# mschoenb97/po2_quantization

Measured on AMD Instinct MI355X. Metric: quantized-conv fwd images/sec, ResNet56 224×224 bs=256; 1/2/4/8 MI355X, higher is better.
Workload: dtype fp32(bf16x3); 1 GPU; resnet56 quantized-conv chain: 56 fused po2-4bit quantize+conv fwd + head (stage-1 and stage-2 conv1->conv2 pairs as one launch each) (stride-2 conv1 + 1x1 shortcut of stages 2-3 as one launch each) (weight packs of the single-conv layers batched: one launch per 36); conv_pairs=True, conv_pairs_stage2=True, s2ds=True, pack_batch=True, autotune=True, image=224, batch_per_gpu=256, global_batch=256, quantizer=po2, bits=4, precision=bf16x3, parallelism=dp1, world_size=1, hip_graph=False

## Files before the change

### po2_quantization_amd/csrc/po2q_conv_rowsk.hip

```cpp
#include <hip/hip_runtime.h>

#include <algorithm>
#include <climits>
#include <cstdlib>
#include <type_traits>
#include <vector>

#include "po2q_epi.h"
#include "po2q_internal.h"
#include "po2q_quant_dev.h"
#include "po2q_rows_dev.h"
#include "po2q_x3_dev.h"

namespace po2q {

namespace {

constexpr int kKSW = 32;
constexpr int kKWC = kKSW + 2;
template <int C> constexpr int kKPlane = kKWC * C * 2;
template <int C> constexpr int kKRawInt = C * kKSW * 4;
template <int C> constexpr int kKRawSlot = kKRawInt<C> + 4 * 256;
template <int C> constexpr int kKTile = C * kKSW * 4;
template <int C, int PD, bool TT>
constexpr int kKLds = 2 * 3 * kKPlane<C> + PD * kKRawSlot<C> + (TT ? 2 * kKTile<C> : 0);

template <int C>
__device__ __forceinline__ int k_addr(int hc, int oct) {
    if constexpr (C == 64)
        return hc * 128 + ((oct ^ (hc & 7)) << 4);
    else
        return x_addr<32>(hc, oct);
}

}

struct RowsKArgs {
    int N, H, W, P, Q;
    int RB, nseg, nstrip, items;
    int remap;
    const float* ps;
    const float* pb;
    int act;
    const float* res;
    WQuant q;
};

template <int C, int PD, bool TT, bool RES, bool NTL>
__device__ __forceinline__ void loader_wave(const float* __restrict__ x, const RowsKArgs& a, unsigned char* raw,
                                            unsigned char* resb, int n, int q0, int p0, int nrows, int rbe) {
    constexpr int NI = C / 8 + 1;
    static_assert(2 * C <= 64, "one halo instruction per row");
    const int lane = threadIdx.x & 63;
    const int HW = a.H * a.W;
    const uint32_t cstride = (uint32_t)HW * 4u;
    const __amdgpu_buffer_rsrc_t rs = rows_rsrc(x + (int64_t)n * C * HW, C * HW * 4);
    const int gq4 = q0 + 4 * (lane & 7);
    const bool qi_ok = gq4 < a.W;
    const uint32_t vi0 = (uint32_t)(lane >> 3) * cstride + (uint32_t)gq4 * 4u;
    const int hside = lane / C, hch = lane % C;
    const int gqh = hside ? q0 + kKSW : q0 - 1;
    const bool qh_ok = gqh >= 0 && gqh < a.W;
    const uint32_t vh0 = (uint32_t)hch * cstride + (uint32_t)gqh * 4u;
    const uint32_t raw_lds = (uint32_t)(uintptr_t)raw;
    const int PQ = a.P * a.Q;
    const __amdgpu_buffer_rsrc_t rr = rows_rsrc(RES ? a.res + (int64_t)n * C * PQ : x, RES ? C * PQ * 4 : 4);
    const uint32_t vr0 = (uint32_t)(lane >> 3) * (uint32_t)PQ * 4u + (uint32_t)gq4 * 4u;
    auto lres = [&](int js) __attribute__((always_inline)) {
        const int orow = js - 3;
        const bool ok = orow >= 0 && orow < rbe && gq4 < a.Q;
        const uint32_t vo = ok ? vr0 + (uint32_t)(p0 + orow) * (uint32_t)a.Q * 4u : 0x7fffffffu;
        const uint32_t base = (uint32_t)(uintptr_t)resb + (uint32_t)((js & 1) * kKTile<C>);
#pragma unroll
        for (int i = 0; i < C / 8; ++i) rows_dma16(rr, vo, i * 8u * (uint32_t)PQ * 4u, base + (uint32_t)i * 1024u);
    };
    auto lrow = [&](int sl, int j) __attribute__((always_inline)) {
        const int h = p0 - 1 + j;
        const bool hok = j < nrows && h >= 0 && h < a.H;
        const uint32_t roff = (uint32_t)(hok ? h : 0) * (uint32_t)a.W * 4u;
        const uint32_t vo = (hok && qi_ok) ? vi0 + roff : 0x7fffffffu;
        const uint32_t base = raw_lds + (uint32_t)(sl * kKRawSlot<C>);
#pragma unroll
        for (int i = 0; i < C / 8; ++i) rows_dma16<NTL>(rs, vo, i * 8u * cstride, base + (uint32_t)i * 1024u);
        rows_dma4<NTL>(rs, (hok && qh_ok) ? vh0 + roff : 0x7fffffffu, base + (uint32_t)kKRawInt<C>);
    };
#pragma unroll
    for (int r = 0; r < PD; ++r) lrow(r, r);
    rows_wait<(PD - 1) * NI>();
    __builtin_amdgcn_s_barrier();
    const int steps = (nrows + 2) / 3 * 3;
    int sl = 0;
    for (int j = 0; j < steps; ++j) {
        rows_wait<(PD - 2) * NI>();
        __builtin_amdgcn_s_barrier();
        if constexpr (RES) lres(j + 1);
        lrow(sl, j + PD);
        sl = sl + 1 == PD ? 0 : sl + 1;
    }
    if (TT && nrows % 3 == 0) {
        if constexpr (RES) rows_wait<0>();
        __builtin_amdgcn_s_barrier();
    }
    asm volatile("s_waitcnt vmcnt(0)" ::: "memory");
}

template <int C, int PD, bool TT, bool LW, bool EPI = false, int DBG = 0, int NTS = 0, bool RES = false,
          bool FP = false, bool PIPE = false>
__global__ __launch_bounds__(LW ? kThreads + 64 : kThreads, C == 64 ? (TT ? 2 : 3) : 4) void conv_rowsk(const float* __restrict__ x, const uint4* __restrict__ wpk,
                                                          const float* __restrict__ scale_p,
                                                          const float* __restrict__ bias, float* __restrict__ y,
                                                          RowsKArgs a) {
    static_assert(!PIPE || (!LW && !RES && !FP && DBG == 0), "pipelined split: plain MFMA-wave plans");
#ifndef PO2Q_ROWSK_FPF
#define PO2Q_ROWSK_FPF 0
#endif
    constexpr bool FPF = PO2Q_ROWSK_FPF != 0 && TT;
    constexpr int K = C;
    constexpr int NCH = C / 32;
    constexpr int KSC = 3 * NCH;
    constexpr int WN = K / 16;
    constexpr int NGW = 2 * WN / 4;
    constexpr int DPW = C / 32;
    constexpr int HPW = C / 2;
    constexpr int PL = kKPlane<C>;
    constexpr int RAWI = kKRawInt<C>;
    constexpr int RAWS = kKRawSlot<C>;
    extern __shared__ __attribute__((aligned(16))) unsigned char lds[];
    const int tid = threadIdx.x, lane = tid & 63;
    const int wave = __builtin_amdgcn_readfirstlane(tid >> 6);
    const int wn = wave % WN;
    const int g0 = (wave / WN) * NGW;
    unsigned char* planes = lds;
    unsigned char* raw = lds + 2 * 3 * PL;
    unsigned char* tile = raw + PD * kKRawSlot<C>;
    unsigned char* resb = tile + 2 * kKTile<C>;

    int blk = blockIdx.x;
    if (a.remap) blk = (blk & 7) * (int)(gridDim.x >> 3) + (blk >> 3);
    const int item = blk;
    if (item >= a.items) return;
    const int strip = item % a.nstrip;
    const int t0 = item / a.nstrip;
    const int seg = t0 % a.nseg;
    const int n = t0 / a.nseg;
    const int q0 = strip * kKSW;
    const int p0 = seg * a.RB;
    const int rbe = min(a.RB, a.P - p0);
    const int nrows = rbe + 2;

    if constexpr (LW) {
        if (wave == 4) {
            loader_wave<C, PD, TT, RES, (NTS & 2) != 0>(x, a, raw, resb, n, q0, p0, nrows, rbe);
            return;
        }
    }

    static_assert(!(FP && LW), "the loader wave keeps its own barrier count");
    bf16x8 bw[3][KSC];
    float scale;
    if constexpr (FP) {
        unsigned* red = reinterpret_cast<unsigned*>(raw);
        unsigned* thr = red + 16;
        bool fin;
        scale = wq_prologue(a.q, thr, red, 4, fin);
        uint4* fr = reinterpret_cast<uint4*>(planes);
        static_assert(KSC * WN * 64 * 16 <= 2 * 3 * PL, "fragment scratch in the planes");
#pragma unroll
        for (int r = 0; r < 3; ++r) {
            wq_pack_tap_row_lds<C>(a.q, C, 32, WN, KSC, r, scale, fin, thr, fr);
#pragma unroll
            for (int ks = 0; ks < KSC; ++ks) bw[r][ks] = __builtin_bit_cast(bf16x8, fr[(ks * WN + wn) * 64 + lane]);
            __syncthreads();
        }
    } else {
#pragma unroll
        for (int r = 0; r < 3; ++r)
#pragma unroll
            for (int ks = 0; ks < KSC; ++ks)
                bw[r][ks] = __builtin_bit_cast(bf16x8, wpk[((r * KSC + ks) * WN + wn) * 64 + lane]);
        scale = *scale_p;
    }
    const int kout = 16 * wn + (lane & 15);
    float bk = bias ? bias[kout] : 0.0f;
    float eps_ = (EPI && a.ps) ? a.ps[kout] : 1.0f;
    float epb_ = (EPI && a.pb) ? a.pb[kout] : 0.0f;
#pragma unroll
    for (int r = 0; r < 3; ++r)
#pragma unroll
        for (int ks = 0; ks < KSC; ++ks) asm volatile("s_waitcnt vmcnt(0)" : "+v"(bw[r][ks]));
    asm volatile("s_waitcnt vmcnt(0)" : "+v"(bk), "+v"(eps_), "+v"(epb_));
    auto outv = [&](float accv) __attribute__((always_inline)) {
        const float v = accv * scale + bk;
        if constexpr (EPI && RES)
            return v * eps_ + epb_;
        else if constexpr (EPI)
            return epi_act(v * eps_ + epb_, a.act);
        else
            return v;
    };

    const int HW = a.H * a.W;
    const uint32_t cstride = (uint32_t)HW * 4u;
    const __amdgpu_buffer_rsrc_t rs = rows_rsrc(x + (int64_t)n * C * HW, C * HW * 4);
    const int cb = lane & 7;
    const int gq4 = q0 + 4 * cb;
    const bool qi_ok = gq4 < a.W;
    const uint32_t vi0 = (uint32_t)((C / 4) * wave + (lane >> 3)) * cstride + (uint32_t)gq4 * 4u;
    const uint32_t soff1 = 8u * cstride;
    const int hv = HPW * wave + lane;
    const int hside = hv / C, hch = hv % C;
    const int gqh = hside ? q0 + kKSW : q0 - 1;
    const bool qh_ok = lane < HPW && gqh >= 0 && gqh < a.W;
    const uint32_t vh0 = (uint32_t)hch * cstride + (uint32_t)gqh * 4u;
    const uint32_t raw_lds = (uint32_t)(uintptr_t)raw;

    const int sc = lane & 31, so = lane >> 5;
    const bool sl_ok = so < DPW;
    const int oct = DPW * wave + (sl_ok ? so : 0);
    const int rd0 = (8 * oct) * (kKSW * 4) + sc * 4;
    const int wa_i = k_addr<C>(sc + 1, oct);
    const int wa_h = k_addr<C>(hside ? kKWC - 1 : 0, hch >> 3) + (hch & 7) * 2;

    int aoff[NGW][KSC];
    {
        const int p = lane & 15, g = lane >> 4;
#pragma unroll
        for (int grp = 0; grp < NGW; ++grp)
#pragma unroll
            for (int ch = 0; ch < NCH; ++ch)
#pragma unroll
                for (int s = 0; s < 3; ++s)
                    aoff[grp][ch * 3 + s] = k_addr<C>(16 * (g0 + grp) + p + s, 4 * ch + g);
    }

    auto load_row = [&](auto SL_, int j) __attribute__((always_inline)) {
        constexpr int sl = decltype(SL_)::value;
        const int h = p0 - 1 + j;
        const bool hok = j < nrows && h >= 0 && h < a.H;
        const uint32_t roff = (uint32_t)(hok ? h : 0) * (uint32_t)a.W * 4u;
        const uint32_t vo = (hok && qi_ok && !(DBG & 8)) ? vi0 + roff : 0x7fffffffu;
        const uint32_t voh = (hok && qh_ok && !(DBG & 1)) ? vh0 + roff : 0x7fffffffu;
        const uint32_t base = raw_lds + (uint32_t)(sl * RAWS);
#pragma unroll
        for (int i = 0; i < DPW; ++i) rows_dma16<(NTS & 2) != 0>(rs, vo, i * soff1, base + (uint32_t)(DPW * wave + i) * 1024u);
        rows_dma4<(NTS & 2) != 0>(rs, voh, base + (uint32_t)RAWI + (uint32_t)wave * 256u);
    };
    constexpr int NR = (RES && !LW) ? NGW : 0;
    static_assert(!RES || TT, "the residual rides on the TT output tile");
    constexpr int VMW = (PD - 1) * (NR + DPW + 1 + NGW) + NGW;
    constexpr int RW = 2 * (DPW + 1) + NGW + NR;
    const int PQ = a.P * a.Q;
    const __amdgpu_buffer_rsrc_t rres = rows_rsrc(NR ? a.res + (int64_t)n * K * PQ : x, NR ? K * PQ * 4 : 4);
    const uint32_t vr0 = (uint32_t)((K / 4) * wave + (lane >> 3)) * (uint32_t)PQ * 4u + (uint32_t)gq4 * 4u;
    auto load_res = [&](int js) __attribute__((always_inline)) {
        if constexpr (NR != 0) {
            const int orow = js - 3;
            const bool ok = orow >= 0 && orow < rbe && gq4 < a.Q;
            const uint32_t vo = ok ? vr0 + (uint32_t)(p0 + orow) * (uint32_t)a.Q * 4u : 0x7fffffffu;
            const uint32_t base = (uint32_t)(uintptr_t)resb + (uint32_t)((js & 1) * kKTile<C>) +
                                  (uint32_t)((K / 4) * wave) * (kKSW * 4u);
#pragma unroll
            for (int i = 0; i < NR; ++i) rows_dma16(rres, vo, i * 8u * (uint32_t)PQ * 4u, base + (uint32_t)i * 1024u);
        }
    };
    const __amdgpu_buffer_rsrc_t ry = rows_rsrc(y + (int64_t)n * K * PQ, K * PQ * 4);

    auto store_tile = [&](const unsigned char* tr, int o, bool orow, int rslot) __attribute__((always_inline)) {
        const int sb = lane & 7;
        const int q = q0 + 4 * sb;
#pragma unroll
        for (int i = 0; i < NGW; ++i) {
            const int c = (K / 4) * wave + 8 * i + (lane >> 3);
            floatx4 v = floatx4{0.f, 0.f, 0.f, 0.f};
            if constexpr (!(DBG & 256)) v = *reinterpret_cast<const floatx4*>(tr + c * (kKSW * 4) + ((sb ^ (c & 7)) << 4));
            if constexpr (RES) {
                const floatx4 r = *reinterpret_cast<const floatx4*>(resb + rslot * kKTile<C> + c * (kKSW * 4) + 16 * sb);
#pragma unroll
                for (int e = 0; e < 4; ++e) v[e] = epi_act(v[e] + r[e], a.act);
            }
            const uint32_t vo = (uint32_t)c * (uint32_t)PQ + (uint32_t)(orow ? o : 0) * a.Q + (uint32_t)q;
            rows_store<(NTS & 1) != 0 || (DBG & 32) != 0>(ry, (orow && q < a.Q && !(DBG & 16)) ? vo * 4u : 0x7fffffffu, v);
        }
    };

    auto split_row = [&](const unsigned char* rw, unsigned char* pb) __attribute__((always_inline)) {
        uint32_t b8[8];
#pragma unroll
        for (int e = 0; e < 8; ++e) b8[e] = *reinterpret_cast<const uint32_t*>(rw + rd0 + e * (kKSW * 4));
        uint4 hi, mid, lo;
        split3(b8, hi, mid, lo);
        if (sl_ok) {
            *reinterpret_cast<uint4*>(pb + wa_i) = hi;
            *reinterpret_cast<uint4*>(pb + PL + wa_i) = mid;
            *reinterpret_cast<uint4*>(pb + 2 * PL + wa_i) = lo;
        }
        if (lane < HPW) {
            uint16_t h16, m16, l16;
            const int hoff = LW ? 4 * (HPW * wave + lane) : wave * 256 + 4 * lane;
            split1(*reinterpret_cast<const uint32_t*>(rw + RAWI + hoff), h16, m16, l16);
            *reinterpret_cast<uint16_t*>(pb + wa_h) = h16;
            *reinterpret_cast<uint16_t*>(pb + PL + wa_h) = m16;
            *reinterpret_cast<uint16_t*>(pb + 2 * PL + wa_h) = l16;
        }
    };

    floatx4 acc[3][NGW];
#pragma unroll
    for (int sl = 0; sl < 3; ++sl)
#pragma unroll
        for (int grp = 0; grp < NGW; ++grp) acc[sl][grp] = floatx4{0.f, 0.f, 0.f, 0.f};

    auto step = [&](auto S_, int j) __attribute__((always_inline)) {
        constexpr int S6 = decltype(S_)::value;
        constexpr int S = S6 % 3;
        constexpr int B2 = S6 % 2;
        constexpr int RS = S6 % PD;
        unsigned char* pb = planes + B2 * 3 * PL;
        [[maybe_unused]] const unsigned char* rw = raw + RS * RAWS;
        if constexpr (LW || PIPE) {
        } else if constexpr (DBG & 64) {
            rows_wait<31>();
        } else {
            rows_wait<VMW>();
        }
        if constexpr (!PIPE) {
            if constexpr (!(DBG & 4)) split_row(rw, pb);
            asm volatile("s_waitcnt lgkmcnt(0)" ::: "memory");
            __builtin_amdgcn_s_barrier();
            if constexpr (!(DBG & 128) && !LW) {
                load_res(j + 1);
                load_row(std::integral_constant<int, RS>{}, j + PD);
            }
        }
        auto fin = [&]() __attribute__((always_inline)) {
            if constexpr (PIPE) {
                asm volatile("s_waitcnt lgkmcnt(0)" ::: "memory");
                __builtin_amdgcn_s_barrier();
                load_row(std::integral_constant<int, (S6 + 1) % PD>{}, j + 1 + PD);
            }
        };
        constexpr int SL[3] = {(S + 1) % 3, S, (S + 2) % 3};
        auto mma = [&](auto G_, auto&& after0) __attribute__((always_inline)) {
            constexpr bool G = decltype(G_)::value;
            bf16x8 af[2][3][NGW];
            auto ldf = [&](bf16x8 (&f)[3][NGW], int ks) __attribute__((always_inline)) {
#pragma unroll
                for (int pl = 0; pl < 3; ++pl)
#pragma unroll
                    for (int grp = 0; grp < NGW; ++grp)
                        f[pl][grp] = __builtin_bit_cast(bf16x8, *reinterpret_cast<const uint4*>(pb + pl * PL + aoff[grp][ks]));
            };
            if constexpr (FPF && !(DBG & 2)) ldf(af[0], 0);
#pragma unroll
            for (int ks = 0; ks < KSC && !(DBG & 2); ++ks) {
                bf16x8 (&cf)[3][NGW] = af[FPF ? (ks & 1) : 0];
                if constexpr (FPF) {
                    if (ks + 1 < KSC) ldf(af[(ks + 1) & 1], ks + 1);
                } else {
                    ldf(cf, ks);
                }
#pragma unroll
                for (int rr = 0; rr < 3; ++rr) {
                    if (G && (j - rr < 0 || j - rr >= rbe)) continue;
#pragma unroll
                    for (int pl = 0; pl < 3; ++pl)
#pragma unroll
                        for (int grp = 0; grp < NGW; ++grp)
                            acc[SL[rr]][grp] = __builtin_amdgcn_mfma_f32_16x16x32_bf16(cf[pl][grp], bw[rr][ks],
                                                                                      acc[SL[rr]][grp], 0, 0, 0);
                }
                if (ks == 0) after0();
            }
        };
        if constexpr (PIPE) {
            auto nxt = [&]() __attribute__((always_inline)) {
                rows_wait<(PD - 1) * (DPW + 1 + NGW)>();
                split_row(raw + ((S6 + 1) % PD) * RAWS, planes + (1 - B2) * 3 * PL);
            };
            if (j >= 2 && j < rbe)
                mma(std::false_type{}, nxt);
            else
                mma(std::true_type{}, nxt);
        } else {
            auto none = []() __attribute__((always_inline)) {};
            if (j >= 2 && j < rbe)
                mma(std::false_type{}, none);
            else
                mma(std::true_type{}, none);
        }
        constexpr int D = (S + 2) % 3;
        if constexpr (TT) {
            if constexpr (NR != 0) rows_wait<RW>();
            store_tile(tile + (1 - B2) * kKTile<C>, p0 + j - 3, j >= 3 && j - 3 < rbe, B2);
            unsigned char* tw = tile + B2 * kKTile<C>;
#pragma unroll
            for (int grp = 0; grp < NGW; ++grp) {
                floatx4 v;
                v[0] = outv(acc[D][grp][0]);
                v[1] = outv(acc[D][grp][1]);
                v[2] = outv(acc[D][grp][2]);
                v[3] = outv(acc[D][grp][3]);
                const int bi = 4 * (g0 + grp) + (lane >> 4);
                if constexpr (!(DBG & 256))
                    *reinterpret_cast<floatx4*>(tw + kout * (kKSW * 4) + ((bi ^ (kout & 7)) << 4)) = v;
                acc[D][grp] = floatx4{0.f, 0.f, 0.f, 0.f};
            }
            fin();
            return;
        }
        const int o = p0 + j - 2;
        const bool orow = j >= 2 && o < p0 + rbe;
        const uint32_t yk = (uint32_t)kout * (uint32_t)PQ + (uint32_t)(orow ? o : 0) * a.Q;
#pragma unroll
        for (int grp = 0; grp < NGW; ++grp) {
            const int q = q0 + 16 * (g0 + grp) + 4 * (lane >> 4);
            floatx4 v;
            v[0] = outv(acc[D][grp][0]);
            v[1] = outv(acc[D][grp][1]);
            v[2] = outv(acc[D][grp][2]);
            v[3] = outv(acc[D][grp][3]);
            rows_store<(NTS & 1) != 0>(ry, (orow && q < a.Q && !(DBG & 16)) ? (yk + (uint32_t)q) * 4u : 0x7fffffffu, v);
            acc[D][grp] = floatx4{0.f, 0.f, 0.f, 0.f};
        }
        fin();
    };

    {
        const floatx4 z = floatx4{0.f, 0.f, 0.f, 0.f};
        auto pre = [&](auto R_) __attribute__((always_inline)) {
            load_res(decltype(R_)::value - PD + 1);
            load_row(R_, decltype(R_)::value);
#pragma unroll
            for (int i = 0; i < NGW; ++i) rows_store<(NTS & 1) != 0>(ry, 0x7fffffffu, z);
        };
        if constexpr (LW) {
            __builtin_amdgcn_s_barrier();
        } else {
            pre(std::integral_constant<int, 0>{});
            pre(std::integral_constant<int, 1>{});
            if constexpr (PD >= 3) pre(std::integral_constant<int, 2>{});
            if constexpr (PIPE) {
                rows_wait<VMW>();
                split_row(raw, planes);
                asm volatile("s_waitcnt lgkmcnt(0)" ::: "memory");
                __builtin_amdgcn_s_barrier();
                load_row(std::integral_constant<int, 0>{}, PD);
            }
        }
    }
    for (int j = 0; j < nrows; j += 6) {
        step(std::integral_constant<int, 0>{}, j);
        step(std::integral_constant<int, 1>{}, j + 1);
        step(std::integral_constant<int, 2>{}, j + 2);
        if (j + 3 >= nrows) break;
        step(std::integral_constant<int, 3>{}, j + 3);
        step(std::integral_constant<int, 4>{}, j + 4);
        step(std::integral_constant<int, 5>{}, j + 5);
    }
    if (TT && nrows % 3 == 0) {
        if constexpr (NR != 0) rows_wait<0>();
        asm volatile("s_waitcnt lgkmcnt(0)" ::: "memory");
        __builtin_amdgcn_s_barrier();
        store_tile(tile + ((nrows - 1) & 1) * kKTile<C>, p0 + rbe - 1, true, nrows & 1);
    }
    asm volatile("s_waitcnt vmcnt(0)" ::: "memory");
}

static int rowsk_lds(int C, int pd, bool tt) {
#define PO2Q_L(c, d) \
    if (C == c && pd == d) return tt ? kKLds<c, d, true> : kKLds<c, d, false>;
    PO2Q_L(64, 2) PO2Q_L(64, 3) PO2Q_L(32, 2) PO2Q_L(32, 3)
#undef PO2Q_L
    return 1 << 30;
}

void rowsk_candidates(const ConvPlan& b, int mode, int bits, int fsr, std::vector<PlanCand>& out) {
    if (mode == 0 || b.groups != 1) return;
    if (bits < 1 || bits > 16) return;
    const long lo = (long)fsr - (1L << (bits - 1)), hi = (long)fsr - 1;
    if (lo < -126 || hi > 127) return;
    if (b.R != 3 || b.S != 3 || b.sh != 1 || b.sw != 1 || b.ph != 1 || b.pw != 1 || b.dh != 1 || b.dw != 1) return;
    if (!((b.C == 64 && b.K == 64) || (b.C == 32 && b.K == 32)) || b.Q % 4 != 0) return;
    if ((int64_t)b.C * b.H * b.W * 4 >= (1LL << 31) || (int64_t)b.K * b.P * b.Q * 4 >= (1LL << 31)) return;
    ConvPlan p = b;
    p.kind = KIND_BF16X3_ROWS;
    p.vrx = 1;
    p.CC = 32;
    p.nchunks = b.C / 32;
    p.NT = b.K / 16;
    p.NJ = 2;
    p.TQ = kKSW;
    p.steps = 3 * p.nchunks;
    p.kblocks = 1;
    p.taps = 9;
    p.PS = 0; p.MI = 0; p.pd = 2;
    p.dma_d0 = p.dma_nck = p.dma_ni = p.dma_nw = p.dma_waves = p.dma_ov = 0;
    p.HH = 0; p.WW = p.WWp = kKWC;
    p.SB = 2 * b.C;
    p.plane = b.C == 64 ? kKPlane<64> : kKPlane<32>;
    p.packed_floats = (int64_t)3 * p.steps * p.NT * 64 * 4;
    p.tilesQ = (p.Q + kKSW - 1) / kKSW;
    const int vrxs[3] = {b.C == 64 ? 1 : 3, 2, b.C == 64 ? 0 : 1};
    for (int vrx : vrxs)
        for (int pd : {3, 2}) {
            if (vrx == 0 || (vrx == 3 && pd < 3)) continue;
            ConvPlan c = p;
            c.pd = pd;
            c.vrx = vrx;
            const bool tt = vrx >= 2;
            c.lds_bytes = rowsk_lds(b.C, pd, tt);
            const int per_cu = std::min(b.C == 64 ? (tt ? 2 : 3) : 4, (int)(163840 / c.lds_bytes));
            const int slots = 256 * per_cu;
            std::vector<std::pair<double, int>> rbs;
            for (int rb = 4; rb <= p.P; ++rb) {
                const int nseg = (p.P + rb - 1) / rb;
                if (rb != (p.P + nseg - 1) / nseg) continue;
                const int64_t items = (int64_t)p.N * nseg * p.tilesQ;
                if (items > INT_MAX / 2) continue;
                rbs.push_back({(double)((items + slots - 1) / slots) * (rb + 2), rb});
            }
            std::sort(rbs.begin(), rbs.end());
            for (int i = 0; i < (int)rbs.size() && i < 2; ++i) {
                ConvPlan d = c;
                d.TP = rbs[i].second;
                d.tilesP = (p.P + d.TP - 1) / d.TP;
                const int64_t items = (int64_t)p.N * d.tilesP * d.tilesQ;
                d.blocks = (items + 7) / 8 * 8;
                out.push_back({0.9 + 0.001 * i + (pd == 2 ? 0.01 : 0.0) + (vrx == vrxs[0] ? 0.0 : 0.02), d});
                if (b.C == 64 && vrx == 1) {
                    ConvPlan f = d;
                    f.fp = 1;
                    out.push_back({0.95 + 0.001 * i + (pd == 2 ? 0.01 : 0.0), f});
                }
                if ((b.C == 64 && vrx == 1) || (b.C == 32 && vrx == 3))
                    for (int nts : {1, 2, 3}) {
                        d.nts = nts;
                        out.push_back({0.905 + 0.001 * i + 0.0001 * nts + (pd == 2 ? 0.01 : 0.0), d});
                    }
            }
        }
}

hipError_t launch_conv_rowsk(const ConvPlan& p, const float* x, const uint16_t* packed, const float* scale,
                             const float* bias, float* y, hipStream_t s, const float* ps, const float* pb,
                             int act, bool epi, const WQuant& q) {
    RowsKArgs a;
    a.N = p.N; a.H = p.H; a.W = p.W; a.P = p.P; a.Q = p.Q;
    a.RB = p.TP; a.nseg = p.tilesP; a.nstrip = p.tilesQ;
    a.items = p.N * p.tilesP * p.tilesQ;
    a.remap = (p.blocks % 8 == 0) ? 1 : 0;
    a.ps = ps;
    a.pb = pb;
    a.act = act;
    a.res = nullptr;
    a.q = q;
    if (p.fp) {
        if (!q.w || p.vrx != 1 || p.C != 64 || p.nts) return hipErrorInvalidValue;
#define PO2Q_RKF(d, e)                                                                                     \
    if (p.pd == d && epi == e) {                                                                             \
        hipLaunchKernelGGL((conv_rowsk<64, d, false, false, e, 0, 0, false, true>), dim3((unsigned)p.blocks), \
                           dim3(kThreads), p.lds_bytes, s, x, reinterpret_cast<const uint4*>(packed), scale, bias, y, a); \
        return hipGetLastError();                                                                            \
    }
        PO2Q_RKF(3, false) PO2Q_RKF(2, false) PO2Q_RKF(3, true) PO2Q_RKF(2, true)
#undef PO2Q_RKF
        return hipErrorInvalidValue;
    }
#define PO2Q_RK1(c, d, e, v, tt, lw)                                                                      \
    if (p.C == c && p.pd == d && epi == e && p.vrx == v && !p.nts) {                                         \
        hipLaunchKernelGGL((conv_rowsk<c, d, tt, lw, e>), dim3((unsigned)p.blocks), dim3(kThreads + (lw ? 64 : 0)), \
                           p.lds_bytes, s, x, reinterpret_cast<const uint4*>(packed), scale, bias, y, a);     \
        return hipGetLastError();                                                                            \
    }
#define PO2Q_RKN1(c, d, e, v, tt, lw, nt)                                                                 \
    if (p.C == c && p.pd == d && epi == e && p.vrx == v && p.nts == nt) {                                    \
        hipLaunchKernelGGL((conv_rowsk<c, d, tt, lw, e, 0, nt>), dim3((unsigned)p.blocks),                  \
                           dim3(kThreads + (lw ? 64 : 0)), p.lds_bytes, s, x, reinterpret_cast<const uint4*>(packed), \
                           scale, bias, y, a);                                                               \
        return hipGetLastError();                                                                            \
    }
#define PO2Q_RKN(c, d, e, v, tt, lw) \
    PO2Q_RKN1(c, d, e, v, tt, lw, 1) PO2Q_RKN1(c, d, e, v, tt, lw, 2) PO2Q_RKN1(c, d, e, v, tt, lw, 3)
#define PO2Q_RK(c, d, e) PO2Q_RK1(c, d, e, 1, false, false) PO2Q_RK1(c, d, e, 2, true, false)
    const int pipe = [] {
        const char* e = getenv("PO2Q_ROWSK_PIPE");
        return e ? atoi(e) : -1;
    }();
#define PO2Q_RKP(d, e, v, tt)                                                                                \
    if ((pipe == 1 || (pipe < 0 && v == 1)) && p.C == 64 && p.pd == d && epi == e && p.vrx == v && !p.nts) { \
        hipLaunchKernelGGL((conv_rowsk<64, d, tt, false, e, 0, 0, false, false, true>), dim3((unsigned)p.blocks), \
                           dim3(kThreads), p.lds_bytes, s, x, reinterpret_cast<const uint4*>(packed), scale, bias, y, a); \
        return hipGetLastError();                                                                            \
    }
    PO2Q_RKP(2, false, 2, true) PO2Q_RKP(3, false, 2, true) PO2Q_RKP(2, true, 2, true) PO2Q_RKP(3, true, 2, true)
    PO2Q_RKP(2, false, 1, false) PO2Q_RKP(3, false, 1, false) PO2Q_RKP(2, true, 1, false) PO2Q_RKP(3, true, 1, false)
#undef PO2Q_RKP
#define PO2Q_RKPN1(d, e, nt)                                                                                 \
    if (pipe != 0 && p.C == 64 && p.pd == d && epi == e && p.vrx == 1 && p.nts == nt) {                      \
        hipLaunchKernelGGL((conv_rowsk<64, d, false, false, e, 0, nt, false, false, true>), dim3((unsigned)p.blocks), \
                           dim3(kThreads), p.lds_bytes, s, x, reinterpret_cast<const uint4*>(packed), scale, bias, y, a); \
        return hipGetLastError();                                                                            \
    }
#define PO2Q_RKPN(d, e) PO2Q_RKPN1(d, e, 1) PO2Q_RKPN1(d, e, 2) PO2Q_RKPN1(d, e, 3)
    PO2Q_RKPN(2, false) PO2Q_RKPN(3, false) PO2Q_RKPN(2, true) PO2Q_RKPN(3, true)
#undef PO2Q_RKPN
#undef PO2Q_RKPN1
#ifdef PO2Q_ROWS_DIAG
    if (const char* dv = getenv("PO2Q_ROWSK_DEBUG")) {
        const int dbg = atoi(dv);
#define PO2Q_RKD(c, d, tt, lw, v)                                                                          \
    if (dbg == v && p.C == c && p.pd == d && (p.vrx >= 2) == tt && (p.vrx == 3) == lw) {                   \
        hipLaunchKernelGGL((conv_rowsk<c, d, tt, lw, false, v>), dim3((unsigned)p.blocks), dim3(kThreads + (lw ? 64 : 0)), \
                           p.lds_bytes, s, x, reinterpret_cast<const uint4*>(packed), scale, bias, y, a);    \
        return hipGetLastError();                                                                           \
    }
#define PO2Q_RKDS(v) PO2Q_RKD(32, 3, true, false, v) PO2Q_RKD(32, 3, true, true, v)
        PO2Q_RKDS(6) PO2Q_RKDS(16) PO2Q_RKDS(2) PO2Q_RKDS(1) PO2Q_RKDS(7)
#undef PO2Q_RKDS
#define PO2Q_RKDS(v) PO2Q_RKD(64, 2, true, false, v)
        PO2Q_RKDS(2) PO2Q_RKDS(4) PO2Q_RKDS(6) PO2Q_RKDS(16) PO2Q_RKDS(64) PO2Q_RKDS(128) PO2Q_RKDS(256)
        PO2Q_RKDS(144) PO2Q_RKDS(400) PO2Q_RKDS(404) PO2Q_RKDS(148) PO2Q_RKDS(20) PO2Q_RKDS(132)
#undef PO2Q_RKDS
#undef PO2Q_RKD
    }
#endif
    PO2Q_RK(64, 3, false) PO2Q_RK(64, 2, false) PO2Q_RK(32, 3, false) PO2Q_RK(32, 2, false)
    PO2Q_RK(64, 3, true) PO2Q_RK(64, 2, true) PO2Q_RK(32, 3, true) PO2Q_RK(32, 2, true)
    PO2Q_RK1(32, 3, false, 3, true, true) PO2Q_RK1(32, 3, true, 3, true, true)
    PO2Q_RKN(64, 3, false, 1, false, false) PO2Q_RKN(64, 2, false, 1, false, false)
    PO2Q_RKN(64, 3, true, 1, false, false) PO2Q_RKN(64, 2, true, 1, false, false)
    PO2Q_RKN(32, 3, false, 3, true, true) PO2Q_RKN(32, 3, true, 3, true, true)

#undef PO2Q_RK
#undef PO2Q_RK1
#undef PO2Q_RKN
#undef PO2Q_RKN1
    return hipErrorInvalidValue;
}

static bool rowsk64_res_on() {
    static const bool on = [] {
        const char* e = getenv("PO2Q_ROWSK_RES");
        return !(e && e[0] == '0');
    }();
    return on;
}

bool rowsk_res_ok(const ConvPlan& p) {
    if (p.kind != KIND_BF16X3_ROWS) return false;
    if (p.C == 32 && p.K == 32) return p.vrx == 3 && p.pd == 3 && !p.fp;
    return p.C == 64 && p.K == 64 && (p.vrx == 1 || p.vrx == 2) && rowsk64_res_on();
}

hipError_t launch_conv_rowsk_res(const ConvPlan& p, const float* x, const uint16_t* packed, const float* scale,
                                 const float* bias, float* y, const float* ps, const float* pb, const float* res,
                                 int act, hipStream_t s, const WQuant& q) {
    if (!rowsk_res_ok(p) || !res) return hipErrorInvalidValue;
    RowsKArgs a;
    a.N = p.N; a.H = p.H; a.W = p.W; a.P = p.P; a.Q = p.Q;
    a.RB = p.TP; a.nseg = p.tilesP; a.nstrip = p.tilesQ;
    a.items = p.N * p.tilesP * p.tilesQ;
    a.remap = (p.blocks % 8 == 0) ? 1 : 0;
    a.ps = ps;
    a.pb = pb;
    a.act = act;
    a.res = res;
    a.q = q;
    if (p.C == 64) {
        constexpr size_t lds64 = kKLds<64, 2, true> + 2 * kKTile<64>;
        if (p.fp) {
            if (!q.w) return hipErrorInvalidValue;
            hipLaunchKernelGGL((conv_rowsk<64, 2, true, false, true, 0, 0, true, true>), dim3((unsigned)p.blocks),
                               dim3(kThreads), lds64, s, x, reinterpret_cast<const uint4*>(packed), scale, bias, y, a);
        } else {
            hipLaunchKernelGGL((conv_rowsk<64, 2, true, false, true, 0, 0, true>), dim3((unsigned)p.blocks),
                               dim3(kThreads), lds64, s, x, reinterpret_cast<const uint4*>(packed), scale, bias, y, a);
        }
        return hipGetLastError();
    }
    const size_t lds = p.lds_bytes + 2 * kKTile<32>;
#define PO2Q_RKR(nt)                                                                                         \
    if (p.nts == nt) {                                                                                       \
        hipLaunchKernelGGL((conv_rowsk<32, 3, true, true, true, 0, nt, true>), dim3((unsigned)p.blocks),      \
                           dim3(kThreads + 64), lds, s, x, reinterpret_cast<const uint4*>(packed), scale, bias, y, a); \
        return hipGetLastError();                                                                            \
    }
    PO2Q_RKR(1) PO2Q_RKR(2) PO2Q_RKR(3)
#undef PO2Q_RKR
    if (p.nts != 0) return hipErrorInvalidValue;
    hipLaunchKernelGGL((conv_rowsk<32, 3, true, true, true, 0, 0, true>), dim3((unsigned)p.blocks),
                       dim3(kThreads + 64), lds, s, x, reinterpret_cast<const uint4*>(packed), scale, bias, y, a);
    return hipGetLastError();
}

}
```

Before: 26250 images/s.

## Add 64-column strip variant of rows conv kernel for C=64 stage-3 layers

Adds an SW=64 template path where a single block covers the full output width (Q between 33 and 64) for C=64 convolutions. It drops the halo loads and uses a new raw-slot layout, bf16x3 split and zeroed plane borders. Matching autotune candidates get a favourable prior cost, and the residual launcher now computes its own strip count. The intent is to cut redundant halo traffic and the per-strip weight-load overhead, at the price of more LDS per block and lower occupancy.

```diff
diff --git a/po2_quantization_amd/csrc/po2q_conv_rowsk.hip b/po2_quantization_amd/csrc/po2q_conv_rowsk.hip
--- a/po2_quantization_amd/csrc/po2q_conv_rowsk.hip
+++ b/po2_quantization_amd/csrc/po2q_conv_rowsk.hip
@@ -24,6 +24,9 @@
 template <int C> constexpr int kKTile = C * kKSW * 4;
 template <int C, int PD, bool TT>
 constexpr int kKLds = 2 * 3 * kKPlane<C> + PD * kKRawSlot<C> + (TT ? 2 * kKTile<C> : 0);
+constexpr int kKRawWave64 = 16 * 64 * 4;
+constexpr int kKRawSlot64 = 4 * kKRawWave64;
+constexpr int rowsk_lds64(int Q, int pd) { return 2 * 3 * (Q + 2) * 128 + pd * kKRawSlot64; }
 
 template <int C>
 __device__ __forceinline__ int k_addr(int hc, int oct) {
@@ -37,6 +40,7 @@
 
 struct RowsKArgs {
     int N, H, W, P, Q;
+    int QR;
     int RB, nseg, nstrip, items;
     int remap;
     const float* ps;
@@ -105,12 +109,20 @@
 }
 
 template <int C, int PD, bool TT, bool LW, bool EPI = false, int DBG = 0, int NTS = 0, bool RES = false,
-          bool FP = false, bool PIPE = false>
-__global__ __launch_bounds__(LW ? kThreads + 64 : kThreads, C == 64 ? (TT ? 2 : 3) : 4) void conv_rowsk(const float* __restrict__ x, const uint4* __restrict__ wpk,
+          bool FP = false, bool PIPE = false, int SW = 32>
+__global__ __launch_bounds__(LW ? kThreads + 64 : kThreads, SW == 64 ? 2 : C == 64 ? (TT ? 2 : 3) : 4) void conv_rowsk(const float* __restrict__ x, const uint4* __restrict__ wpk,
                                                           const float* __restrict__ scale_p,
                                                           const float* __restrict__ bias, float* __restrict__ y,
                                                           RowsKArgs a) {
-    static_assert(!PIPE || (!LW && !RES && !FP && DBG == 0), "pipelined split: plain MFMA-wave plans");
+    constexpr bool W64 = SW == 64;
+    static_assert(SW == 32 || SW == 64, "strip width");
+    static_assert(!PIPE || (!LW && !RES && !FP && (DBG == 0 || W64)), "pipelined split: plain MFMA-wave plans");
+    static_assert(!W64 || (C == 64 && PIPE), "64-column strips: C = 64, pipelined split");
+    static_assert(!W64 || !TT, "64-column strips store directly");
+    static_assert(!W64 || !LW, "64-column strips: no loader wave");
+    static_assert(!W64 || !RES, "64-column strips: no residual ring");
+    static_assert(!W64 || !FP, "64-column strips: packed weights only");
+    static_assert(!W64 || (DBG & ~(2 | 8 | 16)) == 0, "64-column strips: DBG 2, 8, 16");
 #ifndef PO2Q_ROWSK_FPF
 #define PO2Q_ROWSK_FPF 0
 #endif
@@ -119,20 +131,22 @@
     constexpr int NCH = C / 32;
     constexpr int KSC = 3 * NCH;
     constexpr int WN = K / 16;
-    constexpr int NGW = 2 * WN / 4;
-    constexpr int DPW = C / 32;
+    constexpr int NGW = (SW / 16) * WN / 4;
+    constexpr int DPW = W64 ? 4 : C / 32;
+    constexpr int HD = W64 ? 0 : 1;
     constexpr int HPW = C / 2;
-    constexpr int PL = kKPlane<C>;
+    constexpr int PLC = kKPlane<C>;
+    const int PL = W64 ? (a.QR + 2) * 128 : PLC;
     constexpr int RAWI = kKRawInt<C>;
-    constexpr int RAWS = kKRawSlot<C>;
+    constexpr int RAWS = W64 ? kKRawSlot64 : kKRawSlot<C>;
     extern __shared__ __attribute__((aligned(16))) unsigned char lds[];
     const int tid = threadIdx.x, lane = tid & 63;
     const int wave = __builtin_amdgcn_readfirstlane(tid >> 6);
     const int wn = wave % WN;
-    const int g0 = (wave / WN) * NGW;
+    const int g0 = W64 ? 0 : (wave / WN) * NGW;
     unsigned char* planes = lds;
     unsigned char* raw = lds + 2 * 3 * PL;
-    unsigned char* tile = raw + PD * kKRawSlot<C>;
+    unsigned char* tile = raw + PD * RAWS;
     unsigned char* resb = tile + 2 * kKTile<C>;
 
     int blk = blockIdx.x;
@@ -143,7 +157,7 @@
     const int t0 = item / a.nstrip;
     const int seg = t0 % a.nseg;
     const int n = t0 / a.nseg;
-    const int q0 = strip * kKSW;
+    const int q0 = strip * SW;
     const int p0 = seg * a.RB;
     const int rbe = min(a.RB, a.P - p0);
     const int nrows = rbe + 2;
@@ -164,7 +178,7 @@
         bool fin;
         scale = wq_prologue(a.q, thr, red, 4, fin);
         uint4* fr = reinterpret_cast<uint4*>(planes);
-        static_assert(KSC * WN * 64 * 16 <= 2 * 3 * PL, "fragment scratch in the planes");
+        static_assert(KSC * WN * 64 * 16 <= 2 * 3 * PLC, "fragment scratch in the planes");
 #pragma unroll
         for (int r = 0; r < 3; ++r) {
             wq_pack_tap_row_lds<C>(a.q, C, 32, WN, KSC, r, scale, fin, thr, fr);
@@ -213,6 +227,21 @@
     const bool qh_ok = lane < HPW && gqh >= 0 && gqh < a.W;
     const uint32_t vh0 = (uint32_t)hch * cstride + (uint32_t)gqh * 4u;
     const uint32_t raw_lds = (uint32_t)(uintptr_t)raw;
+    uint32_t vi64[4] = {0u, 0u, 0u, 0u};
+    if constexpr (W64) {
+        const int q4 = a.QR >> 2;
+#pragma unroll
+        for (int i = 0; i < 4; ++i) {
+            const int u = 64 * i + lane;
+            const int cl = u / q4;
+            vi64[i] = cl < 16 ? (uint32_t)(16 * wave + cl) * cstride + (uint32_t)(u - cl * q4) * 16u : 0x7fffffffu;
+        }
+        if (tid < 96) {
+            const int side = (tid >> 3) & 1;
+            *reinterpret_cast<uint4*>(planes + (tid >> 4) * PL + (side ? (a.Q + 1) * 128 : 0) + (tid & 7) * 16) =
+                uint4{0u, 0u, 0u, 0u};
+        }
+    }
 
     const int sc = lane & 31, so = lane >> 5;
     const bool sl_ok = so < DPW;
@@ -220,6 +249,8 @@
     const int rd0 = (8 * oct) * (kKSW * 4) + sc * 4;
     const int wa_i = k_addr<C>(sc + 1, oct);
     const int wa_h = k_addr<C>(hside ? kKWC - 1 : 0, hch >> 3) + (hch & 7) * 2;
+    const int rd64 = kKRawWave64 * wave + lane * 4;
+    const int wa64[2] = {k_addr<C>(lane + 1, 2 * wave), k_addr<C>(lane + 1, 2 * wave + 1)};
 
     int aoff[NGW][KSC];
     {
@@ -230,7 +261,8 @@
             for (int ch = 0; ch < NCH; ++ch)
 #pragma unroll
                 for (int s = 0; s < 3; ++s)
-                    aoff[grp][ch * 3 + s] = k_addr<C>(16 * (g0 + grp) + p + s, 4 * ch + g);
+                    aoff[grp][ch * 3 + s] = W64 ? k_addr<C>(p + s, 4 * ch + g) + 2048 * grp
+                                                : k_addr<C>(16 * (g0 + grp) + p + s, 4 * ch + g);
     }
 
     auto load_row = [&](auto SL_, int j) __attribute__((always_inline)) {
@@ -241,13 +273,20 @@
         const uint32_t vo = (hok && qi_ok && !(DBG & 8)) ? vi0 + roff : 0x7fffffffu;
         const uint32_t voh = (hok && qh_ok && !(DBG & 1)) ? vh0 + roff : 0x7fffffffu;
         const uint32_t base = raw_lds + (uint32_t)(sl * RAWS);
-#pragma unroll
-        for (int i = 0; i < DPW; ++i) rows_dma16<(NTS & 2) != 0>(rs, vo, i * soff1, base + (uint32_t)(DPW * wave + i) * 1024u);
-        rows_dma4<(NTS & 2) != 0>(rs, voh, base + (uint32_t)RAWI + (uint32_t)wave * 256u);
+        if constexpr (W64) {
+#pragma unroll
+            for (int i = 0; i < DPW; ++i)
+                rows_dma16<(NTS & 2) != 0>(rs, (hok && !(DBG & 8)) ? vi64[i] + roff : 0x7fffffffu, 0u,
+                                           base + (uint32_t)(DPW * wave + i) * 1024u);
+        } else {
+#pragma unroll
+            for (int i = 0; i < DPW; ++i) rows_dma16<(NTS & 2) != 0>(rs, vo, i * soff1, base + (uint32_t)(DPW * wave + i) * 1024u);
+            rows_dma4<(NTS & 2) != 0>(rs, voh, base + (uint32_t)RAWI + (uint32_t)wave * 256u);
+        }
     };
     constexpr int NR = (RES && !LW) ? NGW : 0;
     static_assert(!RES || TT, "the residual rides on the TT output tile");
-    constexpr int VMW = (PD - 1) * (NR + DPW + 1 + NGW) + NGW;
+    constexpr int VMW = (PD - 1) * (NR + DPW + HD + NGW) + NGW;
     constexpr int RW = 2 * (DPW + 1) + NGW + NR;
     const int PQ = a.P * a.Q;
     const __amdgpu_buffer_rsrc_t rres = rows_rsrc(NR ? a.res + (int64_t)n * K * PQ : x, NR ? K * PQ * 4 : 4);
@@ -284,6 +323,23 @@
     };
 
     auto split_row = [&](const unsigned char* rw, unsigned char* pb) __attribute__((always_inline)) {
+        if constexpr (W64) {
+            const int cpitch = a.QR * 4;
+#pragma unroll
+            for (int so = 0; so < 2; ++so) {
+                uint32_t b8[8];
+#pragma unroll
+                for (int e = 0; e < 8; ++e) b8[e] = *reinterpret_cast<const uint32_t*>(rw + rd64 + (8 * so + e) * cpitch);
+                uint4 hi, mid, lo;
+                split3(b8, hi, mid, lo);
+                if (lane < a.Q) {
+                    *reinterpret_cast<uint4*>(pb + wa64[so]) = hi;
+                    *reinterpret_cast<uint4*>(pb + PL + wa64[so]) = mid;
+                    *reinterpret_cast<uint4*>(pb + 2 * PL + wa64[so]) = lo;
+                }
+            }
+            return;
+        }
         uint32_t b8[8];
 #pragma unroll
         for (int e = 0; e < 8; ++e) b8[e] = *reinterpret_cast<const uint32_t*>(rw + rd0 + e * (kKSW * 4));
@@ -371,10 +427,11 @@
                 }
                 if (ks == 0) after0();
             }
+            if constexpr ((DBG & 2) != 0) after0();
         };
         if constexpr (PIPE) {
             auto nxt = [&]() __attribute__((always_inline)) {
-                rows_wait<(PD - 1) * (DPW + 1 + NGW)>();
+                rows_wait<(PD - 1) * (DPW + HD + NGW)>();
                 split_row(raw + ((S6 + 1) % PD) * RAWS, planes + (1 - B2) * 3 * PL);
             };
             if (j >= 2 && j < rbe)
@@ -473,6 +530,8 @@
 #undef PO2Q_L
     return 1 << 30;
 }
+
+constexpr double kSw64Cost = 0.915;
 
 void rowsk_candidates(const ConvPlan& b, int mode, int bits, int fsr, std::vector<PlanCand>& out) {
     if (mode == 0 || b.groups != 1) return;
@@ -500,6 +559,8 @@
     p.plane = b.C == 64 ? kKPlane<64> : kKPlane<32>;
     p.packed_floats = (int64_t)3 * p.steps * p.NT * 64 * 4;
     p.tilesQ = (p.Q + kKSW - 1) / kKSW;
+    const bool sw64_shape = b.C == 64 && b.Q > kKSW && b.Q <= 64;
+    const int rb0 = sw64_shape ? std::min(4, p.P) : 4;
     const int vrxs[3] = {b.C == 64 ? 1 : 3, 2, b.C == 64 ? 0 : 1};
     for (int vrx : vrxs)
         for (int pd : {3, 2}) {
@@ -512,7 +573,7 @@
             const int per_cu = std::min(b.C == 64 ? (tt ? 2 : 3) : 4, (int)(163840 / c.lds_bytes));
             const int slots = 256 * per_cu;
             std::vector<std::pair<double, int>> rbs;
-            for (int rb = 4; rb <= p.P; ++rb) {
+            for (int rb = rb0; rb <= p.P; ++rb) {
                 const int nseg = (p.P + rb - 1) / rb;
                 if (rb != (p.P + nseg - 1) / nseg) continue;
                 const int64_t items = (int64_t)p.N * nseg * p.tilesQ;
@@ -539,6 +600,39 @@
                     }
             }
         }
+    const char* e64 = getenv("PO2Q_ROWSK_SW64");
+    if (b.C != 64 || b.Q <= kKSW || b.Q > 64 || (e64 && e64[0] == '0')) return;
+    for (int pd : {3, 2}) {
+        ConvPlan c = p;
+        c.pd = pd;
+        c.vrx = 1;
+        c.TQ = 64;
+        c.tilesQ = 1;
+        c.WW = c.WWp = b.Q + 2;
+        c.plane = (b.Q + 2) * 128;
+        c.lds_bytes = rowsk_lds64(b.Q, pd);
+        const int per_cu = std::min(2, (int)(163840 / c.lds_bytes));
+        const int slots = 256 * per_cu;
+        std::vector<std::pair<double, int>> rbs;
+        for (int rb = rb0; rb <= p.P; ++rb) {
+            const int nseg = (p.P + rb - 1) / rb;
+            if (rb != (p.P + nseg - 1) / nseg) continue;
+            const int64_t items = (int64_t)p.N * nseg;
+            if (items > INT_MAX / 2) continue;
+            rbs.push_back({(double)((items + slots - 1) / slots) * (rb + 2), rb});
+        }
+        std::sort(rbs.begin(), rbs.end());
+        for (int i = 0; i < (int)rbs.size() && i < 2; ++i) {
+            ConvPlan d = c;
+            d.TP = rbs[i].second;
+            d.tilesP = (p.P + d.TP - 1) / d.TP;
+            d.blocks = ((int64_t)p.N * d.tilesP + 7) / 8 * 8;
+            for (int nts : {0, 1, 2, 3}) {
+                d.nts = nts;
+                out.push_back({kSw64Cost + 0.001 * i + 0.0001 * nts + (pd == 3 ? 0.01 : 0.0), d});
+            }
+        }
+    }
 }
 
 hipError_t launch_conv_rowsk(const ConvPlan& p, const float* x, const uint16_t* packed, const float* scale,
@@ -554,6 +648,38 @@
     a.act = act;
     a.res = nullptr;
     a.q = q;
+    a.QR = (p.Q + 3) / 4 * 4;
+    if (p.TQ == 64) {
+        if (p.C != 64 || p.vrx != 1 || p.fp || p.Q > 64 || p.Q % 4 != 0 || p.tilesQ != 1 ||
+            p.lds_bytes < (size_t)rowsk_lds64(p.Q, p.pd))
+            return hipErrorInvalidValue;
+        auto go = [&](auto kern) -> hipError_t {
+            if (p.lds_bytes > 64 * 1024) {
+                const hipError_t attr = hipFuncSetAttribute(reinterpret_cast<const void*>(kern),
+                                                            hipFuncAttributeMaxDynamicSharedMemorySize, (int)p.lds_bytes);
+                if (attr != hipSuccess) return attr;
+            }
+            hipLaunchKernelGGL(kern, dim3((unsigned)p.blocks), dim3(kThreads), p.lds_bytes, s, x,
+                               reinterpret_cast<const uint4*>(packed), scale, bias, y, a);
+            return hipGetLastError();
+        };
+#ifdef PO2Q_ROWS_DIAG
+        if (const char* dv = getenv("PO2Q_ROWSK_DEBUG")) {
+            const int dbg = atoi(dv);
+#define PO2Q_RK64D(d, v) \
+    if (dbg == v && p.pd == d && !p.nts) return go(conv_rowsk<64, d, false, false, false, v, 0, false, false, true, 64>);
+            PO2Q_RK64D(2, 2) PO2Q_RK64D(2, 24) PO2Q_RK64D(2, 26) PO2Q_RK64D(3, 2) PO2Q_RK64D(3, 24) PO2Q_RK64D(3, 26)
+#undef PO2Q_RK64D
+        }
+#endif
+#define PO2Q_RK64(d, e, nt) \
+    if (p.pd == d && epi == e && p.nts == nt) return go(conv_rowsk<64, d, false, false, e, 0, nt, false, false, true, 64>);
+#define PO2Q_RK64N(d, e) PO2Q_RK64(d, e, 0) PO2Q_RK64(d, e, 1) PO2Q_RK64(d, e, 2) PO2Q_RK64(d, e, 3)
+        PO2Q_RK64N(3, false) PO2Q_RK64N(2, false) PO2Q_RK64N(3, true) PO2Q_RK64N(2, true)
+#undef PO2Q_RK64N
+#undef PO2Q_RK64
+        return hipErrorInvalidValue;
+    }
     if (p.fp) {
         if (!q.w || p.vrx != 1 || p.C != 64 || p.nts) return hipErrorInvalidValue;
 #define PO2Q_RKF(d, e)                                                                                     \
@@ -666,14 +792,19 @@
     a.act = act;
     a.res = res;
     a.q = q;
+    a.QR = (p.Q + 3) / 4 * 4;
     if (p.C == 64) {
         constexpr size_t lds64 = kKLds<64, 2, true> + 2 * kKTile<64>;
+        a.nstrip = (p.Q + kKSW - 1) / kKSW;
+        a.items = p.N * p.tilesP * a.nstrip;
+        const unsigned blocks = (unsigned)(((int64_t)a.items + 7) / 8 * 8);
+        a.remap = 1;
         if (p.fp) {
             if (!q.w) return hipErrorInvalidValue;
-            hipLaunchKernelGGL((conv_rowsk<64, 2, true, false, true, 0, 0, true, true>), dim3((unsigned)p.blocks),
+            hipLaunchKernelGGL((conv_rowsk<64, 2, true, false, true, 0, 0, true, true>), dim3(blocks),
                                dim3(kThreads), lds64, s, x, reinterpret_cast<const uint4*>(packed), scale, bias, y, a);
         } else {
-            hipLaunchKernelGGL((conv_rowsk<64, 2, true, false, true, 0, 0, true>), dim3((unsigned)p.blocks),
+            hipLaunchKernelGGL((conv_rowsk<64, 2, true, false, true, 0, 0, true>), dim3(blocks),
                                dim3(kThreads), lds64, s, x, reinterpret_cast<const uint4*>(packed), scale, bias, y, a);
         }
         return hipGetLastError();
```

Measured after the change: 26260 images/s (median of 3 runs). About the same (+0.0%).
